# boomluo02/EEMFlow

Measured on AMD Instinct MI355X. Metric: frames/sec + EPE, EEMFlow 1280×720 dt1, 1/2/4/8 MI355X, higher is better.
Workload: dtype f32; 1 GPU; EEMFlow inference, HREM 1280x720 dt1, batch=1 per GPU (BASELINE configs[1]); synthetic 20%-dense voxel pairs resident in HBM, seeded Kaiming weights; height=720, width=1280, batch_per_gpu=1, hip_graph=True, streams_per_gpu=2, coalesced_frames=10, frames_in_flight_hint=2, preheat_steps=200, input_pairs_rotated=8, input_bytes_rotated=294912000, parallelism=replicas x1: frames sharded over ranks, no data-path collective

## Files before the change

eemflow_amd/csrc/api.hip:

```cpp
#include <stdarg.h>
#include <stdlib.h>
#include <string.h>

#include <string>
#include <vector>

#include "ctx.h"
#include <mutex>

static thread_local char g_err[512] = "";
thread_local int eem_last_grid_blocks = 0, eem_last_grid_threads = 0, eem_last_pipe = 0;

void eem_set_error(const char* fmt, ...) {
    va_list ap;
    va_start(ap, fmt);
    vsnprintf(g_err, sizeof(g_err), fmt, ap);
    va_end(ap);
}

extern "C" const char* eemflow_last_error(void) { return g_err; }
extern "C" int eemflow_abi_version(void) { return 1; }

extern "C" int eemflow_create(int device, eemflow_ctx** out) {
    EEM_REQUIRE(out != nullptr, "eemflow_create: out is NULL");
    int ndev = 0;
    EEM_HIP_CHECK(hipGetDeviceCount(&ndev));
    EEM_REQUIRE(device >= 0 && device < ndev, "eemflow_create: device %d of %d", device, ndev);
    EEM_HIP_CHECK(hipSetDevice(device));
    hipDeviceProp_t prop;
    EEM_HIP_CHECK(hipGetDeviceProperties(&prop, device));
    EEM_REQUIRE(strncmp(prop.gcnArchName, "gfx950", 6) == 0,
                "this library is built for gfx950 (MI355X) only; device %d is %s", device, prop.gcnArchName);
    eemflow_ctx* c = new eemflow_ctx();
    c->device = device;
// ... 729 lines not shown
```

eemflow_amd/csrc/common.h:

```cpp
#pragma once
#include <hip/hip_runtime.h>
#include <cstdio>
#include <cstdlib>
#include <stdint.h>
#include <stdio.h>

#include <type_traits>

#include "switch.h"
#include "../../include/eemflow_hip.h"

typedef float f32x2 __attribute__((ext_vector_type(2)));
typedef float f32x4 __attribute__((ext_vector_type(4)));
typedef float f32x16 __attribute__((ext_vector_type(16)));
typedef double f64x2 __attribute__((ext_vector_type(2)));
typedef unsigned u32x4 __attribute__((ext_vector_type(4)));

#define EEM_OK 0
#define EEM_ERR_ARG 1
#define EEM_ERR_HIP 2
#define EEM_ERR_STATE 3

void eem_set_error(const char* fmt, ...);

// ... 1 lines not shown
extern thread_local const char* eem_launch_form;
extern thread_local int eem_launch_jobs;

#define EEM_HIP_CHECK(expr)                                                            \
    do {                                                                               \
        hipError_t _e = (expr);                                                        \
        if (_e != hipSuccess) {                                                        \
            eem_set_error("%s failed: %s (%s:%d)", #expr, hipGetErrorString(_e),       \
                          __FILE__, __LINE__);                                         \
            return EEM_ERR_HIP;                                                        \
        }                                                                              \
    } while (0)

#define EEM_REQUIRE(cond, ...)                                                         \
    do {                                                                               \
        if (!(cond)) {                                                                 \
            eem_set_error(__VA_ARGS__);                                                \
            return EEM_ERR_ARG;                                                        \
        }                                                                              \
    } while (0)

__host__ __device__ static inline int ceil_div(int a, int b) { return (a + b - 1) / b; }

extern thread_local int eem_last_grid_blocks, eem_last_grid_threads, eem_last_pipe;
#define EEM_NOTE_GRID(blocks, threads) do { eem_last_grid_blocks = (int)(blocks); eem_last_grid_threads = (int)(threads); } while (0)
#define EEM_NOTE_PIPE(p) do { eem_last_pipe = (int)(p); } while (0)

template <int I, int N, class F>
__device__ __forceinline__ void static_for(F&& f) {
    if constexpr (I < N) {
        f(std::integral_constant<int, I>{});
        static_for<I + 1, N>(f);
    }
}
template <int N>
__device__ __forceinline__ void wait_vmcnt() {
    asm volatile("s_waitcnt vmcnt(%0)" ::"n"(N > 63 ? 63 : N) : "memory");
}

__device__ static inline unsigned xcd_logical_block(unsigned bid, unsigned nblocks_padded) {
    const unsigned cpx = nblocks_padded >> 3;
    return (bid & 7u) * cpx + (bid >> 3);
}

template <int CTRL>
__device__ static __forceinline__ float dpp_add(float v) {
    return v + __int_as_float(__builtin_amdgcn_update_dpp(0, __float_as_int(v), CTRL, 0xF, 0xF, true));
}
template <int SW>
// ... 65 lines not shown
    float* out;
    int nimg;
    int nimg0;
    int hin, win;
    int hout, wout;
    int hraw, wraw;
    int pad_top, pad_left;
    int act;
    const float* gate;
    int tiles_x, tiles_y;
    float* pool_partial;
    int pool_k;
    const void* const* io;
    int io_frames = 0;
    int in_norm = 0;
    int reverse = 0;
    int nt_store = 0;
    int blocks_per_xcd = 0;
    int wino_f4 = 0;
    const float* ws2r = nullptr;
    const float* res = nullptr;
    const float* wbx3 = nullptr;
    int no_store = 0;
};
#define ENC_ARGS_NOW(a)                                                                                                                  \
    asm volatile("" ::"s"((a).in0), "s"((a).in1), "s"((a).wpk), "s"((a).wpk2), "s"((a).wwino), "s"((a).zero_page), "s"((a).trash),        \
                 "s"((a).bias), "s"((a).out), "s"((a).nimg), "s"((a).nimg0), "s"((a).hin), "s"((a).win), "s"((a).hout), "s"((a).wout),      \
                 "s"((a).hraw), "s"((a).wraw), "s"((a).pad_top), "s"((a).pad_left), "s"((a).act), "s"((a).gate), "s"((a).tiles_x),        \
                 "s"((a).tiles_y), "s"((a).pool_partial), "s"((a).io), "s"(gridDim.x))
int enc_conv_launch(int cin, int cout, int stride, const EncConvArgs& a, hipStream_t stream);
bool enc1_supported(const EncConvArgs& a);
int enc1_launch(const EncConvArgs& a, hipStream_t stream);
bool enc2_supported(int cin, int cout, int stride, int win);
size_t enc2_packed_floats(int cin, int cout);
void enc2_pack_weights(const float* w, int cin, int cout, float* packed);
int enc_conv2_launch(int cin, int cout, int stride, const EncConvArgs& a, hipStream_t stream);
bool s2_supported(int cin, int cout, int stride, const EncConvArgs& a);
int s2_launch(int cin, const EncConvArgs& a, hipStream_t stream);
void enc2_tile(int cin, int cout, int* th, int* tw, int* poolk);
bool s2r_shape(int cin, int cout, int stride);
size_t s2r_packed_floats(int cin, int cout);
int s2r_transform_launch(const float* w, int cin, int cout, float* packed, hipStream_t stream);
bool s2r_supported(int cin, int cout, int stride, const EncConvArgs& a);
int s2r_launch(int cin, const EncConvArgs& a, hipStream_t stream);
bool bx3_shape(int cin, int cout, int stride);
size_t bx3_packed_floats(int cin, int cout);
// ... 137 lines not shown
```

eemflow_amd/csrc/conv_wino4.hip:

```cpp
#include <type_traits>

#include "common.h"

namespace {

#define LDS_PTR(p) ((__attribute__((address_space(3))) void*)(p))
#define GLB_PTR(p) ((const __attribute__((address_space(1))) void*)(p))

template <int C, int NGX, int NGY>
struct W4Cfg {
    static constexpr int WAVES = 8;
    static constexpr int COG = C / 16;
    static constexpr int NG = WAVES / COG;
    static constexpr int TW = NGX * 32, TH = NGY * 8;
    static constexpr int KS = C / 4;
    static constexpr int IN_ROWS = TH + 2;
    static constexpr int ROWP = TW + 8;
    static constexpr int PPR = ROWP / 4;
    static constexpr int PC = IN_ROWS * PPR;
    static constexpr int PLANE_P = (PC + 15) / 16 * 16;
    static constexpr int PLANE = PLANE_P * 4;
    static constexpr int INP = 4 * PLANE_P;
    static constexpr int UP = COG * 9 * 64;
    static constexpr int NI = (INP + UP + 511) / 512;
    static constexpr int STAGE = NI * 2048;
    static constexpr int R = 3;
    static_assert(NG * COG == WAVES && NGX * NGY == NG, "wave roles");
    static_assert((4 * ROWP) % 64 == 32, "the two tile rows of a group must sit 128 bytes apart modulo 256 (ds_read_b128 banks)");
    static_assert((5 * ROWP + 8) * 4 < 65536, "ds_read immediate range");
};

#include "wino4_xf.h"

#ifdef EEM_STAMPS
__device__ unsigned long long g_stamps4[1024 * 8 * 64];
#define STAMP4(i) do { if (C == EEM_STAMPS && lane == 0 && blockIdx.x < 1024 && (i) < 64) g_stamps4[(blockIdx.x * 8 + wave) * 64 + (i)] = __builtin_amdgcn_s_memtime(); } while (0)
#else
#define STAMP4(i)
#endif

template <int C, int NGX, int NGY, int POOLK, int EPI>
__global__ __launch_bounds__(512, 2) void wino4_kernel(EncConvArgs a) {
    ENC_ARGS_NOW(a);
    using K = W4Cfg<C, NGX, NGY>;
    constexpr int R = K::R, NI = K::NI, KS = K::KS;
    constexpr int NWX = POOLK > 0 ? K::TW / POOLK : 1;
    constexpr int RED1 = POOLK > 0 ? NGY * C * NWX : 0;
    constexpr int NSTORE = EPI == 3 ? 0 : 16;
    static_assert(EPI != 3 || POOLK > 0, "a store-free launch needs the pooling output");
    constexpr int NPOOL = POOLK > 0 ? 1 : 0;
    static_assert((R * K::STAGE + 2 * RED1) * 4 <= 160 * 1024, "LDS budget");
    static_assert(POOLK == 0 || (POOLK % 8 == 0 && K::TW % POOLK == 0 && C * NWX * NGY <= 512 && POOLK <= 32), "pool windows");
    static_assert(NI + NSTORE + NPOOL <= 63, "vmcnt immediate");
    __shared__ __attribute__((aligned(256))) float lds[R * K::STAGE + 2 * RED1];
    float* red0 = lds + R * K::STAGE;

    const int tid = threadIdx.x;
    const int lane = tid & 63;
    const int wave = __builtin_amdgcn_readfirstlane(tid >> 6);
    const int j = lane & 15, g = lane >> 4;
    const int tx = j & 7, ty = j >> 3;
    const int cog = wave % K::COG, grp = wave / K::COG;
    const int gx = grp % NGX, gy = grp / NGX;

    STAMP4(0);
#ifdef EEM_STAMPS
    const unsigned long long rt0 = __builtin_amdgcn_s_memrealtime();
#endif
    TileRange tr_ = block_tile_range(a.tiles_x * a.tiles_y * a.nimg, blockIdx.x, gridDim.x);
    int walk_stride = 1;
    if (a.reverse == 3) {
        const int T = a.tiles_x * a.tiles_y * a.nimg;
        const int cpx = (T + 7) >> 3, xcd = blockIdx.x & 7, kb = blockIdx.x >> 3, gb = gridDim.x >> 3;
        const int r0 = xcd * cpx, r1 = min(r0 + cpx, T);
        const int have = r1 - r0 - kb;
        tr_.first = r0 + kb;
        tr_.count = have > 0 ? (have + gb - 1) / gb : 0;
        walk_stride = gb;
// ... 3 lines not shown
    const int total = ntile * KS;
    const int T_all = a.tiles_x * a.tiles_y * a.nimg;
    auto coord_of = [&](int lt) {
        if (a.reverse == 2) return TileCoord{(lt / a.tiles_y) % a.tiles_x, lt % a.tiles_y, lt / (a.tiles_x * a.tiles_y)};
        return tile_coord(a.reverse == 1 ? T_all - 1 - lt : lt, a.tiles_x, a.tiles_y);
    };
    TileCoord cur = coord_of(tr_.first), nxt = cur, prv = cur;
    auto step_tile = [&](TileCoord& t) {
        if (a.reverse == 3) {
            t.bx += walk_stride;
            while (t.bx >= a.tiles_x) { t.bx -= a.tiles_x; if (++t.by == a.tiles_y) { t.by = 0; ++t.n; } }
        } else if (a.reverse == 2) {
            if (++t.by == a.tiles_y) { t.by = 0; if (++t.bx == a.tiles_x) { t.bx = 0; ++t.n; } }
        } else if (a.reverse == 1) tile_retreat(t, a.tiles_x, a.tiles_y);
        else tile_advance(t, a.tiles_x, a.tiles_y);
    };
    const char* zero_page = reinterpret_cast<const char*>(a.zero_page);
    const int plane_in = a.hin * a.win;

    unsigned poff[NI];
    int pryq[NI];
#pragma unroll
    for (int k = 0; k < NI; ++k) {
        const int p = (k * 8 + wave) * 64 + lane;
        if (p < K::INP) {
            const int c = p / K::PLANE_P;
            int rem = p - c * K::PLANE_P;
            const bool pad = rem >= K::PC;
            rem = pad ? K::PC - 1 : rem;
            const int ry = rem / K::PPR, q = rem - ry * K::PPR;
            poff[k] = (unsigned)((c * a.hin + ry) * a.win + q * 4) * 4u;
            pryq[k] = ry | (q << 8) | (pad ? 1 << 16 : 0);
        } else {
            const int up = p - K::INP;
            poff[k] = (unsigned)(up < K::UP ? up : K::UP - 1) * 16u;
            pryq[k] = 1 << 17;
        }
    }
    const char* wbase = reinterpret_cast<const char*>(a.wwino);
    int dma_s = 0;
    int dma_slot = 0;
    unsigned okm = 0;
    bool dma_interior = false;
    const char* dsrc = nullptr;
    auto dma_tile = [&]() {
        const int gy0 = nxt.by * K::TH - 1, gxa = nxt.bx * K::TW - 4;
        dma_interior = gy0 >= 0 && gy0 + K::IN_ROWS <= a.hin && gxa >= 0 && gxa + K::ROWP <= a.win;
        dsrc = reinterpret_cast<const char*>(a.in0 + (size_t)nxt.n * C * plane_in) + ((long)gy0 * a.win + gxa) * 4;
// ... 10 lines not shown
        }
    };
    auto dma_issue = [&]() {
        float* sbase = lds + dma_slot * K::STAGE;
#ifdef EEM_DIAG
        const char* usrc = wbase + (size_t)(a.nt_store & 2 ? 0 : dma_s) * (K::UP * 16);
#else
        const char* usrc = wbase + (size_t)dma_s * (K::UP * 16);
#endif
#pragma unroll
        for (int k = 0; k < NI; ++k) {
            const bool all_in = (k + 1) * 512 <= K::INP, all_u = k * 512 >= K::INP;
            const char* gp;
            if (all_in) gp = dsrc + poff[k];
            else if (all_u) gp = usrc + poff[k];
            else gp = (pryq[k] >= (1 << 17) ? usrc : dsrc) + poff[k];
            if (!all_u && !dma_interior) gp = (okm >> k) & 1 ? gp : zero_page;
            __builtin_amdgcn_global_load_lds(GLB_PTR(gp), LDS_PTR(sbase + (k * 8 + wave) * 256), 16, 0, 0);
        }
        dsrc += (size_t)plane_in * 16;
        if (++dma_s == KS) { dma_s = 0; step_tile(nxt); dma_tile(); }
        if (++dma_slot == R) dma_slot = 0;
    };

    f32x4 biasq;
#pragma unroll
    for (int r = 0; r < 4; ++r) biasq[r] = a.bias[cog * 16 + g * 4 + r];

    const int lbase = g * K::PLANE + (gy * 8 + ty * 4) * K::ROWP + (gx * 8 + tx) * 4 + 2;
    const int wlbase = K::INP * 4 + (cog * 9 * 64 + lane) * 4;

    f32x4 acc[36];
    int L = 0;
    int slot = 0;

    const int prow = (a.hout + 7) >> 3;
    const bool pf_act = tid < NGY * C * NWX;
    const int pf_gy = pf_act ? tid / (C * NWX) : 0;
    const int pf_co = pf_act ? (tid - pf_gy * C * NWX) / NWX : 0, pf_wx = pf_act ? tid % NWX : 0;

    auto step = [&](auto s0_tag, auto waitn_tag) {
        constexpr bool S0 = decltype(s0_tag)::value;
        constexpr int WAITN = decltype(waitn_tag)::value;
        if (L + 1 < total) asm volatile("s_waitcnt vmcnt(%0)" ::"n"(WAITN) : "memory");
        else asm volatile("s_waitcnt vmcnt(0)" ::: "memory");
        if constexpr (S0 && POOLK > 0) asm volatile("s_waitcnt lgkmcnt(0)" ::: "memory");
        __builtin_amdgcn_s_barrier();
        STAMP4(2 + 2 * L);
        if constexpr (S0 && POOLK > 0) {
            if (L > 0) {
                const float* redp = red0 + (((L / KS) - 1) & 1) * RED1;
                const float s = redp[(pf_gy * C + pf_co) * NWX + pf_wx];
                float* pb = a.pool_partial + ((size_t)prv.n * C * prow + prv.by * NGY) * (a.tiles_x * NWX) + prv.bx * NWX;
                float* p = pf_act && prv.by * NGY + pf_gy < prow ? pb + ((size_t)pf_co * prow + pf_gy) * (a.tiles_x * NWX) + pf_wx : a.trash + lane * 4;
                *p = s;
            }
        }
        if (L + R - 1 < total) dma_issue();

        const float* sl = lds + slot * K::STAGE;
        f32x2 t05[6], t12[6], t34[6];
        {
            const float* p = sl + lbase;
            f32x2 pout[6];
            f32x4 pmid[6];
#pragma unroll
            for (int r = 0; r < 6; ++r) {
                pout[r] = f32x2{p[r * K::ROWP + 1], p[r * K::ROWP + 6]};
                pmid[r] = *reinterpret_cast<const f32x4*>(p + r * K::ROWP + 2);
            }
            f32x2 x[6];
#pragma unroll
            for (int r = 0; r < 6; ++r) x[r] = pout[r];
            bt6(x, t05);
#pragma unroll
            for (int r = 0; r < 6; ++r) x[r] = f32x2{pmid[r][0], pmid[r][1]};
            bt6(x, t12);
#pragma unroll
            for (int r = 0; r < 6; ++r) x[r] = f32x2{pmid[r][2], pmid[r][3]};
            bt6(x, t34);
        }
        const f32x4* wl = reinterpret_cast<const f32x4*>(sl + wlbase);
        constexpr int RB = 3;
        f32x4 wq0 = wl[0], wq1 = wl[64];
#pragma unroll
        for (int xb = 0; xb < 6; xb += RB) {
            float v[RB * 6];
#pragma unroll
            for (int xi = 0; xi < RB; ++xi) bt6_row(t05[xb + xi], t12[xb + xi], t34[xb + xi], v + xi * 6);
            __builtin_amdgcn_sched_barrier(0);
#pragma unroll
            for (int pp = 0; pp < RB * 6; ++pp) {
                const int p = xb * 6 + pp;
                if (pp > 0 && (p & 3) == 0) {
                    wq0 = wq1;
                    if ((p >> 2) + 1 < 9) wq1 = wl[((p >> 2) + 1) * 64];
                }
                if constexpr (S0) {
                    const f32x4 z = {0.f, 0.f, 0.f, 0.f};
                    acc[p] = __builtin_amdgcn_mfma_f32_16x16x4f32(wq0[p & 3], v[pp], p == 7 ? biasq : z, 0, 0, 0);
                } else {
                    acc[p] = __builtin_amdgcn_mfma_f32_16x16x4f32(wq0[p & 3], v[pp], acc[p], 0, 0, 0);
                }
            }
            __builtin_amdgcn_sched_barrier(0);
        }
        STAMP4(3 + 2 * L);
        ++L;
        slot = slot + 1 == R ? 0 : slot + 1;
    };

    auto output = [&](int it) {
        const int hw = a.hout * a.wout;
        const int oy = cur.by * K::TH + gy * 8 + ty * 4, ox = cur.bx * K::TW + (gx * 8 + tx) * 4;
        const int co0 = cog * 16 + g * 4;
        float* dst = a.out + (size_t)cur.n * C * hw;
        const float* gsrc = EPI == 1 ? a.gate + (size_t)cur.n * C * hw : nullptr;
        const float* rsrc = EPI == 2 ? a.res + (size_t)cur.n * C * hw : nullptr;
        const bool full = cur.by * K::TH + K::TH <= a.hout && cur.bx * K::TW + K::TW <= a.wout;
        const bool inx = ox < a.wout;
        const unsigned lane_bo = (unsigned)((co0 * a.hout + oy) * a.wout + ox) * 4u;
        float psum[4];
#pragma unroll
        for (int h = 0; h < 2; ++h) {
            f32x2 u[6][4];
#pragma unroll
            for (int xi = 0; xi < 6; ++xi) {
                f32x2 m[6];
#pragma unroll
                for (int nu = 0; nu < 6; ++nu) m[nu] = f32x2{acc[xi * 6 + nu][2 * h], acc[xi * 6 + nu][2 * h + 1]};
                at6(m, u[xi]);
            }
// ... 59 lines not shown
                        if (a.nt_store) __builtin_nontemporal_store(o[yy], reinterpret_cast<f32x4*>(rb + lane_bo + (size_t)yy * a.wout * 4));
                        else *reinterpret_cast<f32x4*>(rb + lane_bo + (size_t)yy * a.wout * 4) = o[yy];
                    } else {
                        float* p = in ? reinterpret_cast<float*>(rb + lane_bo + (size_t)yy * a.wout * 4) : a.trash + lane * 4;
                        *reinterpret_cast<f32x4*>(p) = o[yy];
                    }
                    const float rs = (o[yy][0] + o[yy][1]) + (o[yy][2] + o[yy][3]);
                    ps += (full || in) ? rs : 0.f;
                }
                psum[r] = ps;
            }
        }
        if constexpr (POOLK > 0) {
            constexpr int SW = POOLK / 4;
            float* red = red0 + (it & 1) * RED1;
#pragma unroll
            for (int r = 0; r < 4; ++r) {
                const float sred = window_sum<SW>(psum[r]);
                if ((tx & (SW - 1)) == 0 && ty == 0) red[(gy * C + co0 + r) * NWX + (gx * 8 + tx) / SW] = sred;
            }
        }
    };

    dma_tile();
#pragma unroll
    for (int q = 0; q < R - 1; ++q)
        if (q < total) dma_issue();
    STAMP4(1);

    using T = std::true_type;
    using F = std::false_type;
    for (int it = 0; it < ntile; ++it) {
        if (it == 0) {
            step(T{}, std::integral_constant<int, NI>{});
            step(F{}, std::integral_constant<int, NI>{});
        } else {
            step(T{}, std::integral_constant<int, NI + NSTORE>{});
            step(F{}, std::integral_constant<int, NI + NSTORE + NPOOL>{});
        }
#pragma unroll 1
        for (int s = 2; s < KS; ++s) step(F{}, std::integral_constant<int, NI>{});
        output(it);
        prv = cur;
        step_tile(cur);
    }
    STAMP4(60);
#ifdef EEM_STAMPS
    if (C == EEM_STAMPS && lane == 0 && blockIdx.x < 1024) g_stamps4[(blockIdx.x * 8 + wave) * 64 + 61] = __builtin_amdgcn_s_memrealtime() - rt0;
#endif
    if constexpr (POOLK > 0) {
        asm volatile("s_waitcnt lgkmcnt(0)" ::: "memory");
        __builtin_amdgcn_s_barrier();
        const float* redp = red0 + ((ntile - 1) & 1) * RED1;
        if (pf_act && prv.by * NGY + pf_gy < prow)
            a.pool_partial[(((size_t)prv.n * C + pf_co) * prow + prv.by * NGY + pf_gy) * (a.tiles_x * NWX) + prv.bx * NWX + pf_wx] =
                redp[(pf_gy * C + pf_co) * NWX + pf_wx];
    }
}

struct W4WtJobs { const float* w[W4_WT_JOBS]; float* out[W4_WT_JOBS]; int c[W4_WT_JOBS]; int flip[W4_WT_JOBS]; };
__global__ void wino4_wt_kernel(W4WtJobs jobs) {
    const float* __restrict__ w = jobs.w[blockIdx.y];
    float* __restrict__ out = jobs.out[blockIdx.y];
    const int c = jobs.c[blockIdx.y], transpose_flip = jobs.flip[blockIdx.y];
    const int t = blockIdx.x * blockDim.x + threadIdx.x;
    if (t >= c * c) return;
    const int co = t / c, ci = t - co * c;
    float gk[3][3];
    for (int ky = 0; ky < 3; ++ky)
        for (int kx = 0; kx < 3; ++kx)
            gk[ky][kx] = transpose_flip ? w[((size_t)ci * c + co) * 9 + (2 - ky) * 3 + (2 - kx)]
// ... 26 lines not shown
template <int C>
int launch4_c(const EncConvArgs& a0, hipStream_t stream) {
    using W = W4Tile<C>;
    using K = W4Cfg<C, W::NGX, W::NGY>;
    EncConvArgs a = a0;
    a.tiles_x = ceil_div(a.wout, K::TW);
    a.tiles_y = ceil_div(a.hout, K::TH);
    const int T = a.tiles_x * a.tiles_y * a.nimg;
    int per_xcd = ceil_div(T, 8);
    static const int env_cap = enc_blocks_per_xcd(C == 16 ? "F16" : (C == 32 ? "F32" : "F64"), 0);
    int cap = env_cap > 0 ? env_cap : 32;
    if (env_cap <= 0 && a.blocks_per_xcd > 0 && C == 16 && per_xcd > 16) cap = (per_xcd + 1) / 2;
    if (per_xcd > cap) per_xcd = cap;
    if (a.pool_partial != nullptr && a.pool_k != W::POOLK) {
        eem_set_error("wino4: fused pooling with k=%d is not built for C=%d", a.pool_k, C);
        return EEM_ERR_ARG;
    }
    EEM_NOTE_GRID(per_xcd * 8, 512);
    EEM_NOTE_PIPE(2);
    if ((a.gate != nullptr || a.res != nullptr) && (a.pool_partial != nullptr || (a.gate != nullptr && a.res != nullptr))) {
        eem_set_error("wino4: gate / residual epilogues come without pooling and one at a time");
        return EEM_ERR_ARG;
    }
    if (a.pool_partial != nullptr && a.no_store && C == 64)
        hipLaunchKernelGGL((wino4_kernel<C, W::NGX, W::NGY, W::POOLK, (C == 64 ? 3 : 0)>), dim3(per_xcd * 8), dim3(512), 0, stream, a);
    else if (a.pool_partial != nullptr)
        hipLaunchKernelGGL((wino4_kernel<C, W::NGX, W::NGY, W::POOLK, 0>), dim3(per_xcd * 8), dim3(512), 0, stream, a);
    else if (a.gate != nullptr)
        hipLaunchKernelGGL((wino4_kernel<C, W::NGX, W::NGY, 0, 1>), dim3(per_xcd * 8), dim3(512), 0, stream, a);
    else if (a.res != nullptr)
        hipLaunchKernelGGL((wino4_kernel<C, W::NGX, W::NGY, 0, 2>), dim3(per_xcd * 8), dim3(512), 0, stream, a);
    else
        hipLaunchKernelGGL((wino4_kernel<C, W::NGX, W::NGY, 0, 0>), dim3(per_xcd * 8), dim3(512), 0, stream, a);
    EEM_HIP_CHECK(hipGetLastError());
    return EEM_OK;
}

}

#ifdef EEM_STAMPS
extern "C" __attribute__((visibility("default"))) int eemflow_debug_read_stamps4(unsigned long long* dst, size_t n) {
    return hipMemcpyFromSymbol(dst, HIP_SYMBOL(g_stamps4), n * sizeof(unsigned long long)) == hipSuccess ? 0 : 2;
}
extern "C" __attribute__((visibility("default"))) int eemflow_debug_clear_stamps4() {
    static unsigned long long zero[1024 * 8 * 64];
    return hipMemcpyToSymbol(HIP_SYMBOL(g_stamps4), zero, sizeof zero) == hipSuccess ? 0 : 2;
}
#endif

size_t wino4_packed_floats(int c) { return (size_t)36 * c * c; }

int wino4_transform_multi_launch(const float* const* w, const int* c, const int* transpose_flip, float* const* packed, int njobs,
                                 hipStream_t stream) {
    EEM_REQUIRE(njobs >= 1 && njobs <= W4_WT_JOBS, "wino4_transform_multi_launch: njobs=%d", njobs);
    W4WtJobs J;
    int cmax = 0;
    for (int i = 0; i < W4_WT_JOBS; ++i) {
        const int k = i < njobs ? i : 0;
        EEM_REQUIRE(c[k] == 16 || c[k] == 32 || c[k] == 64, "wino4_transform_multi_launch: C=%d", c[k]);
        J.w[i] = w[k]; J.out[i] = packed[k]; J.c[i] = c[k]; J.flip[i] = transpose_flip[k];
        if (c[k] > cmax) cmax = c[k];
    }
    hipLaunchKernelGGL(wino4_wt_kernel, dim3(ceil_div(cmax * cmax, 256), njobs), dim3(256), 0, stream, J);
    EEM_HIP_CHECK(hipGetLastError());
    return EEM_OK;
}

int wino4_transform_launch(const float* w, int c, int transpose_flip, float* packed, hipStream_t stream) {
// ... 19 lines not shown
```

eemflow_amd/csrc/ctx.h:

```cpp
#pragma once
#include <stdarg.h>
#include <string.h>

#include <string>
#include <vector>

#include "../../include/eemflow_hip.h"
#include "common.h"
#include "gconv.h"
#include "eraft_kernels.h"
#include "wnc.h"

inline constexpr int kTaps53[53] = {0,  2,  4,  6,  8,  10, 12, 14, 16, 18, 20, 21, 22, 23, 24, 26, 28, 29,
                                    30, 31, 32, 33, 34, 36, 38, 39, 40, 41, 42, 44, 46, 47, 48, 49, 50, 51,
                                    52, 54, 56, 57, 58, 59, 60, 62, 64, 66, 68, 70, 72, 74, 76, 78, 80};
constexpr int kNTaps = 53;
constexpr int kDecIn = kNTaps + 16;
constexpr int kDecW = 100;

struct TailW {
    size_t wpk = 0, bias = 0;
    int cin = 0, cout = 0, ksize = 3;
};

// ... 144 lines not shown
struct Hook {
    hipStream_t st = nullptr;
    bool timing = false;
    int reps = 1;
    bool repeat = false;
    int pass = 0;
    size_t slot = 0;
    std::vector<hipEvent_t> evs;
    std::vector<eemflow_kernel_stat> stats;

    static bool skipped(const char* name);

    template <class F>
    int run(const char* name, double flops, double bytes, F&& launch) {
#ifdef EEM_DIAG
        if (skipped(name)) {
            static const float spin = sw_float<SW_EEM_SKIP_SPIN_US>();
            return spin > 0.f ? spin_launch(spin, st) : EEM_OK;
        }
#endif
        if (!timing) return launch(st);
        if (repeat) {
            if (evs.size() < 2) { evs.resize(2, nullptr); EEM_HIP_CHECK(hipEventCreate(&evs[0])); EEM_HIP_CHECK(hipEventCreate(&evs[1])); }
            eem_last_grid_blocks = eem_last_grid_threads = eem_last_pipe = 0;
            int rc = launch(st);
            if (rc != EEM_OK) return rc;
            EEM_HIP_CHECK(hipEventRecord(evs[0], st));
            for (int i = 0; i < reps; ++i)
                if ((rc = launch(st)) != EEM_OK) return rc;
            EEM_HIP_CHECK(hipEventRecord(evs[1], st));
            EEM_HIP_CHECK(hipEventSynchronize(evs[1]));
            float ms = 0.f;
            EEM_HIP_CHECK(hipEventElapsedTime(&ms, evs[0], evs[1]));
            eemflow_kernel_stat ks;
            memset(&ks, 0, sizeof(ks));
            strncpy(ks.name, name, sizeof(ks.name) - 1);
            ks.flops = flops; ks.bytes = bytes; ks.ms = ms;
            ks.blocks = eem_last_grid_blocks;
            ks.pipe = eem_last_pipe;
            stats.push_back(ks);
            return EEM_OK;
        }
        if (evs.size() < 2 * (slot + 1)) {
            evs.resize(2 * (slot + 1), nullptr);
            EEM_HIP_CHECK(hipEventCreate(&evs[2 * slot]));
            EEM_HIP_CHECK(hipEventCreate(&evs[2 * slot + 1]));
        }
        eem_last_grid_blocks = eem_last_grid_threads = eem_last_pipe = 0;
        EEM_HIP_CHECK(hipEventRecord(evs[2 * slot], st));
        const int rc = launch(st);
        if (rc != EEM_OK) return rc;
        EEM_HIP_CHECK(hipEventRecord(evs[2 * slot + 1], st));
        if (pass == 0) {
            eemflow_kernel_stat ks;
            memset(&ks, 0, sizeof(ks));
            strncpy(ks.name, name, sizeof(ks.name) - 1);
            ks.flops = flops; ks.bytes = bytes; ks.ms = 0.f;
            ks.blocks = eem_last_grid_blocks;
            ks.pipe = eem_last_pipe;
            stats.push_back(ks);
        }
        ++slot;
        return EEM_OK;
    }
    int collect(bool count);
    void release();
};

extern thread_local unsigned long g_realloc_events;
int ensure(DevBuf& b, size_t floats);
int refresh_wino(eemflow_ctx* c, hipStream_t);
int ensure_bx3(eemflow_ctx* c, int l, hipStream_t st, const float** w_out);
int ensure_s2r(eemflow_ctx* c, int l, hipStream_t st, const float** w_out);
int ensure_wino(eemflow_ctx* c, int l, int dir, int batch, hipStream_t st, const float** w_out, int* f4_out);
int ensure_dec_wnc(eemflow_ctx* c, hipStream_t st);
int ensure_train_wino(eemflow_ctx* c, int batch, hipStream_t st);
int ensure_forward_wino(eemflow_ctx* c, int batch, hipStream_t st);
void drop_graph(eemflow_ctx* c);
int compute_shape(eemflow_ctx* c, int batch, int in_h, int in_w, int out_h, int out_w, Shape* s, int nimg = -1);
int alloc_workspace(eemflow_ctx* c, const Shape& s);

bool s2r_wanted();
// ... 9 lines not shown
```

eemflow_amd/csrc/schedule.hip:

```cpp
#include "ctx.h"

bool s2r_wanted() { return sw_on<SW_EEM_S2R>(); }
bool bx3_wanted(int l) {
    const EncLayerDesc& d = kEncLayers[l];
    return d.stride == 2 || bx3_s1_wanted(d.cin);
}
bool dec_wnc_wanted(const eemflow_ctx* c, int gw, int batch) {
    const char* e = sw_raw<SW_EEM_DEC_WNC>();
    if (c->dec_wnc == nullptr || gw % 4 != 0 || (e && e[0] == '0')) return false;
    return (e && e[0] == '1') || batch >= 4;
}
static bool tail_head_lds_wanted(const Shape& s, const TailHeadArgs& ha) {
    const char* e = sw_raw<SW_EEM_TAIL_HEAD_LDS>();
    if (s.stream || !tail_head_lds_supported(ha) || (e && e[0] == '0')) return false;
    return (e && e[0] == '1') || s.batch >= 4;
}

static void enc_walk(const eemflow_ctx* c, const Shape& s, int layer, EncConvArgs& a) {
    a.reverse = 0;
    static_assert(kSwitches[SW_EEM_COLWALK].dflt == ((1 << ENC_3_2) | (1 << ENC_3_3)), "switches.def.h: EEM_COLWALK's default");
    const int cw = sw_int_once<SW_EEM_COLWALK>();
    if (s.enc_batch >= 2 && ((cw >> layer) & 1)) a.reverse = 2;
    static_assert(kSwitches[SW_EEM_WALK3].dflt == ((1 << ENC_1_2) | (1 << ENC_2_2) | (1 << ENC_2_3) | (1 << ENC_3_2) | (1 << ENC_3_3)), "switches.def.h: EEM_WALK3's default");
    const int w3 = sw_int_once<SW_EEM_WALK3>();
    if (s.enc_batch >= 2 && ((w3 >> layer) & 1)) a.reverse = 3;
    a.nt_store = 0;
    static const int kInFlightBlocks[ENC_NUM] = {12, 24, 0, 29, 29, 0, 0, 0};
    a.blocks_per_xcd = c->frames_in_flight >= 3 ? kInFlightBlocks[layer] : 0;
}

#ifndef EEM_DIAG
bool Hook::skipped(const char*) { return false; }
#else
// ... 223 lines not shown
        a.zero_page = c->zero_page;
        a.trash = c->zero_page + 256;
        a.bias = c->arena + c->enc_b[sp.layer];
        a.out = sp.out;
        a.nimg = n2; a.nimg0 = sp.layer == ENC_1_1 ? s.nimg0 : n2;
        a.hin = sp.hin; a.win = sp.win; a.hout = sp.hout; a.wout = sp.wout;
        a.hraw = sp.layer == ENC_1_1 ? s.in_h : sp.hin;
        a.wraw = sp.layer == ENC_1_1 ? s.in_w : sp.win;
        a.pad_top = sp.layer == ENC_1_1 ? c->pad[2] : 0;
        a.pad_left = sp.layer == ENC_1_1 ? c->pad[0] : 0;
        if (sp.layer == ENC_1_1 && prepadded != nullptr) {
            a.in0 = prepadded;
            a.in1 = prepadded + (size_t)s.batch * c->cin0 * s.hp * s.wp;
            a.hraw = s.hp; a.wraw = s.wp; a.pad_top = 0; a.pad_left = 0;
        }
        a.act = 1;
        a.gate = nullptr;
        a.pool_partial = nullptr;
        a.pool_k = 0;
        a.io = sp.layer == ENC_1_1 ? io : nullptr;
        a.io_frames = (sp.layer == ENC_1_1 && io != nullptr) ? c->cur_io_frames : 0;
        a.in_norm = (sp.layer == ENC_1_1 && c->deferred_norm && prepadded == nullptr) ? 1 : 0;
        a.no_store = 0;
        enc_walk(c, s, sp.layer, a);
        for (int k = 0; k < 3; ++k)
            if (s.fuse[k] && sp.layer == (k == 0 ? ENC_1_2 : k == 1 ? ENC_2_3 : ENC_3_3)) {
                a.pool_partial = c->ppart[k].p;
                a.pool_k = k == 0 ? 32 : k == 1 ? 16 : 8;
                if (k == 2 && may_skip_store) a.no_store = 1;
            }
        const double opix = (double)n2 * sp.hout * sp.wout;
        const double flops = 2.0 * opix * d.cout * d.cin * 9;
        const double ipix = sp.layer == ENC_1_1 ? (double)n2 * s.in_h * s.in_w : (double)n2 * sp.hin * sp.win;
        const double bytes = 4.0 * (ipix * d.cin + opix * d.cout + (double)d.cout * d.cin * 9 + d.cout);
        rc = hk.run(sp.name, flops, bytes,
                    [&](hipStream_t st) { return enc_conv_launch(d.cin, d.cout, d.stride, a, st); });
        if (rc != EEM_OK) return rc;
    }
    return EEM_OK;
}

int run_enc12(eemflow_ctx* c, const Shape& s, const float* e1, const float* e2, Hook& hk, const void* const* io, const float* prepadded,
              bool* done) {
    *done = false;
    const bool off = !sw_on<SW_EEM_FUSE12>();
    if (off || s.stream || c->deferred_norm || c->keep_stage_stores || c->enc0_generic || prepadded != nullptr || !c->use_wino || !c->enc_wino[ENC_1_2] ||
// ... 150 lines not shown
```

eemflow_amd/csrc/switches.def.h:

```cpp

SW(EEM_WINO,               INT,   1,     LOAD,  "0: direct-convolution kernels; 2: Winograd, never F(4x4)")
SW(EEM_WINO4_LAYERS,       RAW,   0,     LOAD,  "<mask>: f4_mask is always that mask (bit 0/1/2: C = 16/32/64); unset: by batch")
SW(EEM_S2R,                ON1,   0,     CALL,  "the stride-2 layers on conv_s2r.hip")
SW(EEM_BX3_S1,             INT,   0,     CALL,  "<mask>: stride-1 layers on conv_bx3.hip (bit 0: C = 32, 1: C = 64)")
SW(EEM_NO_BX3,             ON1,   0,     CALL,  "no layer on conv_bx3.hip")
SW(EEM_NO_S2W,             ON1,   0,     CALL,  "no layer on conv_s2.hip")
SW(EEM_S2W_64,             ON1,   0,     CALL,  "conv_s2.hip takes 32 -> 64 too")
SW(EEM_NO_ENC1,            PRESENT, 0,   CALL,  "pconv1_1 on the generic encoder kernel instead of conv_enc1.hip")
SW(EEM_V,                  FAMILY, 0,    CALL,  "EEM_V<cin>_<cout>=<index>: conv_enc2.hip's variant of that layer (100 + i: persistent variant i)")
SW(EEM_ENC_PER_XCD,        FAMILY, 0,    ONCE,  "EEM_ENC_PER_XCD[_<tag>]=<n>: blocks per XCD of the persistent encoder kernels, the tagged name first (once per launcher)")
SW(EEM_DEC_WNC,            RAW,   0,     CALL,  "decoders' conv1 / conv5 on conv_wnc.hip - 0: never, 1: at every batch, unset: from batch 4 on")
SW(EEM_TAIL_HEAD_LDS,      RAW,   0,     BUILD, "the tail head's LDS form - 0: never, 1: wherever it is supported, unset: from four frames per launch on")
SW(EEM_FUSE12,             ON1,   0,     BUILD, "pconv1_1 + pconv1_2 as one launch; also read at alloc_workspace for its block scratch")
SW(EEM_COLWALK,            INT,   192,   ONCE,  "<layer mask>: tiles in columns (default: ENC_3_2, ENC_3_3)")
SW(EEM_WALK3,              INT,   218,   ONCE,  "<layer mask>: interleaved tile walk, supersedes EEM_COLWALK (default: every stride-1 layer but pconv1_1)")
SW(EEM_NO_WNC,             ON1,   0,     CALL,  "wnc_supported is false everywhere")
SW(EEM_WNC_SMALL_MAXPX,    LONG,  30000, CALL,  "maps below it take conv_wnc.hip's 4 x 32 block tile")
SW(EEM_NO_TAIL_MULTI,      ON1,   0,     CALL,  "the small-grid conv never takes several tiles per block")
SW(EEM_SKIP_KERNELS,       RAW,   0,     ONCE,  "\"prefix;prefix\": launches skipped by name (the flow is garbage)")
SW(EEM_SKIP_SPIN_US,       FLOAT, 0,     ONCE,  "a skipped launch holds its place in the stream that long (once per launch site, Hook::run)")
SW(EEM_SKIP_SPIN_BLOCKS,   INT,   1,     ONCE,  "blocks of the place-holder launch (x 576 threads)")
SW(EEM_SKIP_SPIN_CODE,     ON1,   0,     ONCE,  "the place-holder walks code instead of sleeping")
SW(EEM_SPANS,              ON1,   0,     ONCE,  "encoder / tail chain spans to stderr every 64 frames")
SW(EEM_E12_DBG,            INT,   0,     CALL,  "enc12_kernel - 1: no phase A, 2: no phase B, 4: A's stores to the trash page, 8: A without MFMAs")
SW(EEM_WG_DBG,             INT,   0,     ONCE,  "copied to the wgrad kernels' debug word (once per launcher instantiation)")
// ... 64 lines not shown
```

Before: 10940 frames/s.

## Share Winograd input transforms across waves via LDS in 64-channel F(4x4) conv

Adds a shared-V variant of the Winograd F(4x4) kernel for 64-channel layers. The input tile is transformed once per tile group, with each wave computing half a tile and writing it to a double-buffered V region in LDS, instead of every output-channel wave redoing the same input transform. Weights and raw input now stream through separate LDS buffers with a new DMA plan and vmcnt accounting, and it is enabled by default for cin=64. This trades redundant ALU transform work for extra LDS traffic and a more complex pipeline, with some risk of new stalls. Timing stamps and variant reporting are extended as well.

Result: faster. 11100 frames/s, median of 6 (+1.5%).

```diff
diff --git a/eemflow_amd/csrc/api.hip b/eemflow_amd/csrc/api.hip
--- a/eemflow_amd/csrc/api.hip
+++ b/eemflow_amd/csrc/api.hip
@@ -9,7 +9,7 @@
 #include <mutex>
 
 static thread_local char g_err[512] = "";
-thread_local int eem_last_grid_blocks = 0, eem_last_grid_threads = 0, eem_last_pipe = 0;
+thread_local int eem_last_grid_blocks = 0, eem_last_grid_threads = 0, eem_last_pipe = 0, eem_last_variant = 0;
 
 void eem_set_error(const char* fmt, ...) {
     va_list ap;
diff --git a/eemflow_amd/csrc/common.h b/eemflow_amd/csrc/common.h
--- a/eemflow_amd/csrc/common.h
+++ b/eemflow_amd/csrc/common.h
@@ -47,9 +47,10 @@
 
 __host__ __device__ static inline int ceil_div(int a, int b) { return (a + b - 1) / b; }
 
-extern thread_local int eem_last_grid_blocks, eem_last_grid_threads, eem_last_pipe;
+extern thread_local int eem_last_grid_blocks, eem_last_grid_threads, eem_last_pipe, eem_last_variant;
 #define EEM_NOTE_GRID(blocks, threads) do { eem_last_grid_blocks = (int)(blocks); eem_last_grid_threads = (int)(threads); } while (0)
 #define EEM_NOTE_PIPE(p) do { eem_last_pipe = (int)(p); } while (0)
+#define EEM_NOTE_VARIANT(v) do { eem_last_variant = (int)(v); } while (0)
 
 template <int I, int N, class F>
 __device__ __forceinline__ void static_for(F&& f) {
@@ -161,6 +162,7 @@
     const float* res = nullptr;
     const float* wbx3 = nullptr;
     int no_store = 0;
+    int vshare = 0;
 };
 #define ENC_ARGS_NOW(a)                                                                                                                  \
     asm volatile("" ::"s"((a).in0), "s"((a).in1), "s"((a).wpk), "s"((a).wpk2), "s"((a).wwino), "s"((a).zero_page), "s"((a).trash),        \
diff --git a/eemflow_amd/csrc/conv_wino4.hip b/eemflow_amd/csrc/conv_wino4.hip
--- a/eemflow_amd/csrc/conv_wino4.hip
+++ b/eemflow_amd/csrc/conv_wino4.hip
@@ -33,13 +33,15 @@
 #include "wino4_xf.h"
 
 #ifdef EEM_STAMPS
-__device__ unsigned long long g_stamps4[1024 * 8 * 64];
-#define STAMP4(i) do { if (C == EEM_STAMPS && lane == 0 && blockIdx.x < 1024 && (i) < 64) g_stamps4[(blockIdx.x * 8 + wave) * 64 + (i)] = __builtin_amdgcn_s_memtime(); } while (0)
+__device__ unsigned long long g_stamps4[1024 * 8 * 128];
+#define STAMP4(i) do { if (C == EEM_STAMPS && blockIdx.x < 1024 && (i) < 128) { __builtin_amdgcn_sched_barrier(0); if (lane == 0) g_stamps4[(blockIdx.x * 8 + wave) * 128 + (i)] = __builtin_amdgcn_s_memtime(); __builtin_amdgcn_sched_barrier(0); } } while (0)
+#define STAMP4K(base, L) do { if ((L) < 29) STAMP4((base) + 2 * (L)); } while (0)
 #else
 #define STAMP4(i)
+#define STAMP4K(base, L)
 #endif
 
-template <int C, int NGX, int NGY, int POOLK, int EPI>
+template <int C, int NGX, int NGY, int POOLK, int EPI, bool VS = false>
 __global__ __launch_bounds__(512, 2) void wino4_kernel(EncConvArgs a) {
     ENC_ARGS_NOW(a);
     using K = W4Cfg<C, NGX, NGY>;
@@ -49,11 +51,16 @@
     constexpr int NSTORE = EPI == 3 ? 0 : 16;
     static_assert(EPI != 3 || POOLK > 0, "a store-free launch needs the pooling output");
     constexpr int NPOOL = POOLK > 0 ? 1 : 0;
-    static_assert((R * K::STAGE + 2 * RED1) * 4 <= 160 * 1024, "LDS budget");
+    constexpr int RAWF = K::INP * 4, UF = K::UP * 4, VF = K::NG * 9 * 64 * 4;
+    constexpr int UBASE = 3 * RAWF, VBASE = UBASE + 2 * UF;
+    constexpr int RING = VS ? VBASE + 2 * VF : R * K::STAGE;
+    static_assert(!VS || (K::COG == 4 && (EPI == 0 || EPI == 3) && K::INP + K::UP == NI * 512 && K::UP % 64 == 0 && KS >= 3),
+                  "shared V: four waves per tile group, a piece plan without padding whose wave-instructions are all weights or all input");
+    static_assert((RING + 2 * RED1) * 4 <= 160 * 1024, "LDS budget");
     static_assert(POOLK == 0 || (POOLK % 8 == 0 && K::TW % POOLK == 0 && C * NWX * NGY <= 512 && POOLK <= 32), "pool windows");
     static_assert(NI + NSTORE + NPOOL <= 63, "vmcnt immediate");
-    __shared__ __attribute__((aligned(256))) float lds[R * K::STAGE + 2 * RED1];
-    float* red0 = lds + R * K::STAGE;
+    __shared__ __attribute__((aligned(256))) float lds[RING + 2 * RED1];
+    float* red0 = lds + RING;
 
     const int tid = threadIdx.x;
     const int lane = tid & 63;
@@ -103,8 +110,11 @@
     int pryq[NI];
 #pragma unroll
     for (int k = 0; k < NI; ++k) {
-        const int p = (k * 8 + wave) * 64 + lane;
-        if (p < K::INP) {
+        const int p = VS ? (k * 8 + wave) * 64 + lane - K::UP : (k * 8 + wave) * 64 + lane;
+        if (VS && p < 0) {
+            poff[k] = (unsigned)(p + K::UP) * 16u;
+            pryq[k] = 1 << 17;
+        } else if (p < K::INP) {
             const int c = p / K::PLANE_P;
             int rem = p - c * K::PLANE_P;
             const bool pad = rem >= K::PC;
@@ -161,6 +171,29 @@
         if (++dma_s == KS) { dma_s = 0; step_tile(nxt); dma_tile(); }
         if (++dma_slot == R) dma_slot = 0;
     };
+    const bool raw_hi = (4 * 8 + wave) * 64 >= K::UP;
+    auto dma_issue_vs = [&](bool do_w, bool do_raw, int ws, int uslot) {
+        float* ub = lds + UBASE + uslot * UF;
+        float* rb = lds + dma_slot * RAWF;
+        const char* usrc = wbase + (size_t)ws * (K::UP * 16);
+#pragma unroll
+        for (int k = 0; k < NI; ++k) {
+            const bool all_u = (k + 1) * 512 <= K::UP, all_in = k * 512 >= K::UP;
+            const int pb = (k * 8 + wave) * 64;
+            if (all_u || (!all_in && pb < K::UP)) {
+                if (do_w) __builtin_amdgcn_global_load_lds(GLB_PTR(usrc + poff[k]), LDS_PTR(ub + pb * 4), 16, 0, 0);
+            } else if (do_raw) {
+                const char* gp = dsrc + poff[k];
+                if (!dma_interior) gp = (okm >> k) & 1 ? gp : zero_page;
+                __builtin_amdgcn_global_load_lds(GLB_PTR(gp), LDS_PTR(rb + (pb - K::UP) * 4), 16, 0, 0);
+            }
+        }
+        if (do_raw) {
+            dsrc += (size_t)plane_in * 16;
+            if (++dma_s == KS) { dma_s = 0; step_tile(nxt); dma_tile(); }
+            if (++dma_slot == R) dma_slot = 0;
+        }
+    };
 
     f32x4 biasq;
 #pragma unroll
@@ -185,7 +218,7 @@
         else asm volatile("s_waitcnt vmcnt(0)" ::: "memory");
         if constexpr (S0 && POOLK > 0) asm volatile("s_waitcnt lgkmcnt(0)" ::: "memory");
         __builtin_amdgcn_s_barrier();
-        STAMP4(2 + 2 * L);
+        STAMP4K(2, L);
         if constexpr (S0 && POOLK > 0) {
             if (L > 0) {
                 const float* redp = red0 + (((L / KS) - 1) & 1) * RED1;
@@ -196,6 +229,7 @@
             }
         }
         if (L + R - 1 < total) dma_issue();
+        STAMP4K(64, L);
 
         const float* sl = lds + slot * K::STAGE;
         f32x2 t05[6], t12[6], t34[6];
@@ -219,6 +253,7 @@
             for (int r = 0; r < 6; ++r) x[r] = f32x2{pmid[r][2], pmid[r][3]};
             bt6(x, t34);
         }
+        STAMP4K(65, L);
         const f32x4* wl = reinterpret_cast<const f32x4*>(sl + wlbase);
         constexpr int RB = 3;
         f32x4 wq0 = wl[0], wq1 = wl[64];
@@ -244,9 +279,108 @@
             }
             __builtin_amdgcn_sched_barrier(0);
         }
-        STAMP4(3 + 2 * L);
+        STAMP4K(3, L);
         ++L;
         slot = slot + 1 == R ? 0 : slot + 1;
+    };
+
+    auto duty_half = [&](auto h_tag, int rslot, int vslot) {
+        constexpr int H = decltype(h_tag)::value;
+        const float* p = lds + rslot * RAWF + lbase;
+        f32x2 t05[6], t12[6], t34[6];
+        {
+            f32x2 pout[6];
+            f32x4 pmid[6];
+#pragma unroll
+            for (int r = 0; r < 6; ++r) {
+                pout[r] = f32x2{p[r * K::ROWP + 1], p[r * K::ROWP + 6]};
+                pmid[r] = *reinterpret_cast<const f32x4*>(p + r * K::ROWP + 2);
+            }
+            f32x2 x[6];
+#pragma unroll
+            for (int r = 0; r < 6; ++r) x[r] = pout[r];
+            bt6(x, t05);
+#pragma unroll
+            for (int r = 0; r < 6; ++r) x[r] = f32x2{pmid[r][0], pmid[r][1]};
+            bt6(x, t12);
+#pragma unroll
+            for (int r = 0; r < 6; ++r) x[r] = f32x2{pmid[r][2], pmid[r][3]};
+            bt6(x, t34);
+        }
+        float v[18];
+#pragma unroll
+        for (int xi = 0; xi < 3; ++xi) bt6_row(t05[3 * H + xi], t12[3 * H + xi], t34[3 * H + xi], v + 6 * xi);
+        float* vb = lds + VBASE + vslot * VF + (grp * 9 * 64 + lane) * 4;
+        if constexpr (H == 0) {
+#pragma unroll
+            for (int q = 0; q < 4; ++q) *reinterpret_cast<f32x4*>(vb + q * 256) = f32x4{v[4 * q], v[4 * q + 1], v[4 * q + 2], v[4 * q + 3]};
+            *reinterpret_cast<f32x2*>(vb + 4 * 256) = f32x2{v[16], v[17]};
+        } else {
+            *reinterpret_cast<f32x2*>(vb + 4 * 256 + 2) = f32x2{v[0], v[1]};
+#pragma unroll
+            for (int q = 5; q < 9; ++q) *reinterpret_cast<f32x4*>(vb + q * 256) = f32x4{v[4 * q - 18], v[4 * q - 17], v[4 * q - 16], v[4 * q - 15]};
+        }
+    };
+    auto make_v = [&](int rslot, int vslot) {
+        if ((cog >> 1) == grp) {
+            if (cog & 1) duty_half(std::integral_constant<int, 1>{}, rslot, vslot);
+            else duty_half(std::integral_constant<int, 0>{}, rslot, vslot);
+        }
+    };
+    int uslot = 0;
+    int wnext = 1;
+    auto step_vs = [&](auto s0_tag, auto xtra_tag) {
+        constexpr bool S0 = decltype(s0_tag)::value;
+        constexpr int XTRA = decltype(xtra_tag)::value;
+        constexpr int NR_LO = (NI * 512 - K::UP) / 512, NR_HI = (NI * 512 - K::UP + 511) / 512;
+        if (L + 2 < total) {
+            if (raw_hi) asm volatile("s_waitcnt vmcnt(%0)" ::"n"(NR_HI + XTRA) : "memory");
+            else asm volatile("s_waitcnt vmcnt(%0)" ::"n"(NR_LO + XTRA) : "memory");
+        } else {
+            asm volatile("s_waitcnt vmcnt(0)" ::: "memory");
+        }
+        asm volatile("s_waitcnt lgkmcnt(0)" ::: "memory");
+        __builtin_amdgcn_s_barrier();
+        STAMP4K(2, L);
+        if constexpr (S0 && POOLK > 0) {
+            if (L > 0) {
+                const float* redp = red0 + (((L / KS) - 1) & 1) * RED1;
+                const float s = redp[(pf_gy * C + pf_co) * NWX + pf_wx];
+                float* pb = a.pool_partial + ((size_t)prv.n * C * prow + prv.by * NGY) * (a.tiles_x * NWX) + prv.bx * NWX;
+                float* p = pf_act && prv.by * NGY + pf_gy < prow ? pb + ((size_t)pf_co * prow + pf_gy) * (a.tiles_x * NWX) + pf_wx : a.trash + lane * 4;
+                *p = s;
+            }
+        }
+        if (L + 1 < total) dma_issue_vs(true, L + 3 < total, wnext, uslot ^ 1);
+        STAMP4K(64, L);
+
+        const f32x4* wl = reinterpret_cast<const f32x4*>(lds + UBASE + uslot * UF + (cog * 9 * 64 + lane) * 4);
+        const f32x4* vl = reinterpret_cast<const f32x4*>(lds + VBASE + uslot * VF + (grp * 9 * 64 + lane) * 4);
+        f32x4 wq0 = wl[0], vq0 = vl[0], wq1 = wl[64], vq1 = vl[64];
+        __builtin_amdgcn_sched_barrier(0);
+#pragma unroll
+        for (int p = 0; p < 36; ++p) {
+            if (p > 0 && (p & 3) == 0) {
+                wq0 = wq1; vq0 = vq1;
+                if ((p >> 2) + 1 < 9) { wq1 = wl[((p >> 2) + 1) * 64]; vq1 = vl[((p >> 2) + 1) * 64]; }
+                __builtin_amdgcn_sched_barrier(0);
+            }
+            if constexpr (S0) {
+                const f32x4 z = {0.f, 0.f, 0.f, 0.f};
+                acc[p] = __builtin_amdgcn_mfma_f32_16x16x4f32(wq0[p & 3], vq0[p & 3], p == 7 ? biasq : z, 0, 0, 0);
+            } else {
+                acc[p] = __builtin_amdgcn_mfma_f32_16x16x4f32(wq0[p & 3], vq0[p & 3], acc[p], 0, 0, 0);
+            }
+        }
+        __builtin_amdgcn_sched_barrier(0);
+        STAMP4K(3, L);
+        const int rnext = slot + 1 == R ? 0 : slot + 1;
+        if (L + 1 < total) make_v(rnext, uslot ^ 1);
+        STAMP4K(65, L);
+        ++L;
+        slot = rnext;
+        uslot ^= 1;
+        wnext = wnext + 1 == KS ? 0 : wnext + 1;
     };
 
     auto output = [&](int it) {
@@ -352,14 +486,37 @@
         }
     };
 
+    using T = std::true_type;
+    using F = std::false_type;
+    if constexpr (VS) {
+        (void)wlbase;
+        dma_tile();
+        dma_issue_vs(false, true, 0, 0);
+        dma_issue_vs(true, false, 0, 0);
+        dma_issue_vs(false, true, 0, 0);
+        dma_issue_vs(false, true, 0, 0);
+        if (raw_hi) asm volatile("s_waitcnt vmcnt(%0)" ::"n"(NI + 2) : "memory");
+        else asm volatile("s_waitcnt vmcnt(%0)" ::"n"(NI + 1) : "memory");
+        __builtin_amdgcn_s_barrier();
+        make_v(0, 0);
+        STAMP4(1);
+        for (int it = 0; it < ntile; ++it) {
+            if (it == 0) step_vs(T{}, std::integral_constant<int, 0>{});
+            else step_vs(T{}, std::integral_constant<int, NSTORE>{});
+#pragma unroll 1
+            for (int s = 1; s < KS; ++s) step_vs(F{}, std::integral_constant<int, 0>{});
+            output(it);
+            if (it == 0) STAMP4(62);
+            prv = cur;
+            step_tile(cur);
+        }
+    } else {
     dma_tile();
 #pragma unroll
     for (int q = 0; q < R - 1; ++q)
         if (q < total) dma_issue();
     STAMP4(1);
 
-    using T = std::true_type;
-    using F = std::false_type;
     for (int it = 0; it < ntile; ++it) {
         if (it == 0) {
             step(T{}, std::integral_constant<int, NI>{});
@@ -371,12 +528,14 @@
 #pragma unroll 1
         for (int s = 2; s < KS; ++s) step(F{}, std::integral_constant<int, NI>{});
         output(it);
+        if (it == 0) STAMP4(62);
         prv = cur;
         step_tile(cur);
     }
+    }
     STAMP4(60);
 #ifdef EEM_STAMPS
-    if (C == EEM_STAMPS && lane == 0 && blockIdx.x < 1024) g_stamps4[(blockIdx.x * 8 + wave) * 64 + 61] = __builtin_amdgcn_s_memrealtime() - rt0;
+    if (C == EEM_STAMPS && lane == 0 && blockIdx.x < 1024) g_stamps4[(blockIdx.x * 8 + wave) * 128 + 61] = __builtin_amdgcn_s_memrealtime() - rt0;
 #endif
     if constexpr (POOLK > 0) {
         asm volatile("s_waitcnt lgkmcnt(0)" ::: "memory");
@@ -449,6 +608,19 @@
         eem_set_error("wino4: gate / residual epilogues come without pooling and one at a time");
         return EEM_ERR_ARG;
     }
+    if constexpr (C == 64) {
+        if (a.vshare && a.gate == nullptr && a.res == nullptr) {
+            if (a.pool_partial != nullptr && a.no_store)
+                hipLaunchKernelGGL((wino4_kernel<C, W::NGX, W::NGY, W::POOLK, 3, true>), dim3(per_xcd * 8), dim3(512), 0, stream, a);
+            else if (a.pool_partial != nullptr)
+                hipLaunchKernelGGL((wino4_kernel<C, W::NGX, W::NGY, W::POOLK, 0, true>), dim3(per_xcd * 8), dim3(512), 0, stream, a);
+            else
+                hipLaunchKernelGGL((wino4_kernel<C, W::NGX, W::NGY, 0, 0, true>), dim3(per_xcd * 8), dim3(512), 0, stream, a);
+            EEM_HIP_CHECK(hipGetLastError());
+            EEM_NOTE_VARIANT(1);
+            return EEM_OK;
+        }
+    }
     if (a.pool_partial != nullptr && a.no_store && C == 64)
         hipLaunchKernelGGL((wino4_kernel<C, W::NGX, W::NGY, W::POOLK, (C == 64 ? 3 : 0)>), dim3(per_xcd * 8), dim3(512), 0, stream, a);
     else if (a.pool_partial != nullptr)
@@ -470,7 +642,7 @@
     return hipMemcpyFromSymbol(dst, HIP_SYMBOL(g_stamps4), n * sizeof(unsigned long long)) == hipSuccess ? 0 : 2;
 }
 extern "C" __attribute__((visibility("default"))) int eemflow_debug_clear_stamps4() {
-    static unsigned long long zero[1024 * 8 * 64];
+    static unsigned long long zero[1024 * 8 * 128];
     return hipMemcpyToSymbol(HIP_SYMBOL(g_stamps4), zero, sizeof zero) == hipSuccess ? 0 : 2;
 }
 #endif
diff --git a/eemflow_amd/csrc/ctx.h b/eemflow_amd/csrc/ctx.h
--- a/eemflow_amd/csrc/ctx.h
+++ b/eemflow_amd/csrc/ctx.h
@@ -190,7 +190,7 @@
         if (!timing) return launch(st);
         if (repeat) {
             if (evs.size() < 2) { evs.resize(2, nullptr); EEM_HIP_CHECK(hipEventCreate(&evs[0])); EEM_HIP_CHECK(hipEventCreate(&evs[1])); }
-            eem_last_grid_blocks = eem_last_grid_threads = eem_last_pipe = 0;
+            eem_last_grid_blocks = eem_last_grid_threads = eem_last_pipe = eem_last_variant = 0;
             int rc = launch(st);
             if (rc != EEM_OK) return rc;
             EEM_HIP_CHECK(hipEventRecord(evs[0], st));
@@ -205,7 +205,7 @@
             strncpy(ks.name, name, sizeof(ks.name) - 1);
             ks.flops = flops; ks.bytes = bytes; ks.ms = ms;
             ks.blocks = eem_last_grid_blocks;
-            ks.pipe = eem_last_pipe;
+            ks.pipe = eem_last_pipe; ks.reserved = eem_last_variant;
             stats.push_back(ks);
             return EEM_OK;
         }
@@ -214,7 +214,7 @@
             EEM_HIP_CHECK(hipEventCreate(&evs[2 * slot]));
             EEM_HIP_CHECK(hipEventCreate(&evs[2 * slot + 1]));
         }
-        eem_last_grid_blocks = eem_last_grid_threads = eem_last_pipe = 0;
+        eem_last_grid_blocks = eem_last_grid_threads = eem_last_pipe = eem_last_variant = 0;
         EEM_HIP_CHECK(hipEventRecord(evs[2 * slot], st));
         const int rc = launch(st);
         if (rc != EEM_OK) return rc;
@@ -225,7 +225,7 @@
             strncpy(ks.name, name, sizeof(ks.name) - 1);
             ks.flops = flops; ks.bytes = bytes; ks.ms = 0.f;
             ks.blocks = eem_last_grid_blocks;
-            ks.pipe = eem_last_pipe;
+            ks.pipe = eem_last_pipe; ks.reserved = eem_last_variant;
             stats.push_back(ks);
         }
         ++slot;
diff --git a/eemflow_amd/csrc/schedule.hip b/eemflow_amd/csrc/schedule.hip
--- a/eemflow_amd/csrc/schedule.hip
+++ b/eemflow_amd/csrc/schedule.hip
@@ -9,6 +9,10 @@
     const char* e = sw_raw<SW_EEM_DEC_WNC>();
     if (c->dec_wnc == nullptr || gw % 4 != 0 || (e && e[0] == '0')) return false;
     return (e && e[0] == '1') || batch >= 4;
+}
+static bool w4_vshare_wanted(int cin) {
+    const char* e = sw_raw<SW_EEM_W4_VSHARE>();
+    return cin == 64 && !(e && e[0] == '0');
 }
 static bool tail_head_lds_wanted(const Shape& s, const TailHeadArgs& ha) {
     const char* e = sw_raw<SW_EEM_TAIL_HEAD_LDS>();
@@ -278,6 +282,7 @@
         a.io_frames = (sp.layer == ENC_1_1 && io != nullptr) ? c->cur_io_frames : 0;
         a.in_norm = (sp.layer == ENC_1_1 && c->deferred_norm && prepadded == nullptr) ? 1 : 0;
         a.no_store = 0;
+        a.vshare = w4_vshare_wanted(d.cin) ? 1 : 0;
         enc_walk(c, s, sp.layer, a);
         for (int k = 0; k < 3; ++k)
             if (s.fuse[k] && sp.layer == (k == 0 ? ENC_1_2 : k == 1 ? ENC_2_3 : ENC_3_3)) {
diff --git a/eemflow_amd/csrc/switches.def.h b/eemflow_amd/csrc/switches.def.h
--- a/eemflow_amd/csrc/switches.def.h
+++ b/eemflow_amd/csrc/switches.def.h
@@ -1,6 +1,7 @@
 
 SW(EEM_WINO,               INT,   1,     LOAD,  "0: direct-convolution kernels; 2: Winograd, never F(4x4)")
 SW(EEM_WINO4_LAYERS,       RAW,   0,     LOAD,  "<mask>: f4_mask is always that mask (bit 0/1/2: C = 16/32/64); unset: by batch")
+SW(EEM_W4_VSHARE,          RAW,   0,     CALL,  "conv_wino4.hip's shared-V form - 0: never, 1: wherever it is built (C = 64, plain / store-free epilogues of the EEMFlow forward), unset: on")
 SW(EEM_S2R,                ON1,   0,     CALL,  "the stride-2 layers on conv_s2r.hip")
 SW(EEM_BX3_S1,             INT,   0,     CALL,  "<mask>: stride-1 layers on conv_bx3.hip (bit 0: C = 32, 1: C = 64)")
 SW(EEM_NO_BX3,             ON1,   0,     CALL,  "no layer on conv_bx3.hip")
```
